# jhhung/kISS

Measured on AMD Instinct MI355X. Metric: bases/sec suffix_sort (chm13v2.0-size synthetic, k=256), higher is better.
Workload: dtype u8; 1 GPU; suffix_sort genome-like synthetic n=3117292070 k=256 (stand-in for chm13v2.0.fa, BASELINE.json configs[1]); PARALLEL_SORTING; text resident in HBM, SA left in HBM; n=3117292070, k=256, seed=2, parallelism=single GPU, lms=905939973, lms_rounds=9, tied_after_round0_item_rounds=184319413, big_segment_item_rounds=72866550, workspace_bytes=80357006484, induce_passes=47

## Files before the change

include/kiss_hip.h:

```cpp
#ifndef KISS_HIP_H
#define KISS_HIP_H

#include <stddef.h>
#include <stdint.h>

#ifdef __cplusplus
extern "C" {
#endif

#define KISS_HIP_VERSION 103

typedef enum kiss_hip_status {
    KISS_HIP_OK = 0,
    KISS_HIP_E_INVALID = -1,
    KISS_HIP_E_NO_DEVICE = -2,
    KISS_HIP_E_HIP = -3,
    KISS_HIP_E_NOMEM = -4,
    KISS_HIP_E_UNSUPPORTED = -5,
    KISS_HIP_E_INTERNAL = -6,
    KISS_HIP_E_IO = -7,
    KISS_HIP_E_DEEP = -8
} kiss_hip_status;

#define KISS_HIP_ALGO_PARALLEL_SORTING 0
// ... 141 lines not shown
                             const uint32_t *splitters, int groups, uint64_t *d_keys_out, uint32_t *d_pos_out,
                             void *stream);
int kiss_hip_stage_sort(kiss_hip_ctx *ctx, const uint64_t *d_keys, const uint32_t *d_pos, uint64_t count, uint64_t n,
                        uint32_t k, uint32_t *d_sorted_out, uint32_t *d_ctx_out, void *stream);
int kiss_hip_stage_induce(kiss_hip_ctx *ctx, uint64_t n, uint32_t k, const uint32_t *d_far_sorted,
                          const uint32_t *d_far_ctx, uint64_t m_far, const uint32_t *d_near_pos, uint64_t near_count,
                          const uint64_t counts12[12], uint32_t *d_SA, void *stream);
int kiss_hip_stage_induce_exact(kiss_hip_ctx *ctx, uint64_t n, uint32_t h0, const uint32_t *d_far_sorted,
                                const uint32_t *d_far_ctx, uint64_t m_far, const uint32_t *d_near_pos, uint64_t near_count,
                                const uint64_t counts12[12], uint32_t *d_SA, void *stream, int *exact_out);
int kiss_hip_stage_refine_exact(kiss_hip_ctx *ctx, uint64_t n, uint32_t h0, uint32_t *d_SA, void *stream);

int kiss_hip_debug_radix_sort(kiss_hip_ctx *ctx, uint64_t *keys, uint32_t *pos, uint64_t count, int key_lo_bit);
int kiss_hip_debug_scan_u32(kiss_hip_ctx *ctx, uint32_t *data, uint64_t count);
int kiss_hip_debug_fail_alloc_over(kiss_hip_ctx *ctx, uint64_t bytes);
int kiss_hip_debug_splitters(const uint64_t *hist, uint64_t bins, int groups, uint32_t *splitters_out,
                             uint64_t *group_counts_out);

typedef struct kiss_hip_fmi_view {
    uint64_t n_sa;
    uint32_t cnt[4];
    uint32_t pri;
    uint32_t sa_intv;
    const uint8_t *bwt;
    const uint32_t *occ1;
    const uint8_t *occ2;
    const uint32_t *sa;
    const uint64_t *b;
    const uint32_t *b_occ;
} kiss_hip_fmi_view;
// ... 180 lines not shown
```

kiss_amd/_lib.py:

```python
import ctypes
import os

_HERE = os.path.dirname(os.path.abspath(__file__))
LIB_PATH = os.path.join(_HERE, "libkiss_hip.so")
HOOKS_LIB_PATH = os.path.join(_HERE, "libkiss_hip_hooks.so")

KISS_HIP_OK = 0
KISS_HIP_E_INVALID, KISS_HIP_E_NO_DEVICE, KISS_HIP_E_HIP, KISS_HIP_E_NOMEM = -1, -2, -3, -4
KISS_HIP_E_UNSUPPORTED, KISS_HIP_E_INTERNAL, KISS_HIP_E_IO, KISS_HIP_E_DEEP = -5, -6, -7, -8
ALGO_PARALLEL_SORTING = 0
ALGO_PREFIX_DOUBLING = 1
MAX_N = 4294963200
VIEW_LOCAL_KEYS, VIEW_LOCAL_POS, VIEW_PART_KEYS, VIEW_PART_POS, VIEW_SORTED, VIEW_SORTED_CTX = range(6)

KERNEL_CLASSES = [
    "pack", "classify", "radix_hist", "radix_scatter", "scan", "keygather", "flag_compact",
    "place", "induce_count", "induce_scatter", "induce_small", "fm_query", "fm_build", "segrank",
    "group_heads", "isa",
]


class Stats(ctypes.Structure):
    _fields_ = [
        ("n", ctypes.c_uint64), ("m", ctypes.c_uint64), ("k", ctypes.c_uint32), ("depth", ctypes.c_uint32),
# ... 202 lines not shown
    lib.kiss_hip_ctx_create_sized.argtypes = [ctypes.POINTER(vp), ctypes.c_int, ctypes.c_uint64, ctypes.c_uint64]
    lib.kiss_hip_ctx_release_io_buffers.argtypes = [vp]
    ip = ctypes.POINTER(ctypes.c_int)
    lib.kiss_hip_multi_create.argtypes = [ctypes.POINTER(vp), ip, ctypes.c_int, ctypes.c_uint64]
    lib.kiss_hip_multi_destroy.argtypes = [vp]
    lib.kiss_hip_multi_suffix_sort_dna_u32.argtypes = [vp, vp, ctypes.c_uint64, ctypes.c_uint32, ctypes.c_int, vp]
    lib.kiss_hip_multi_suffix_sort_dna_u32_dev.argtypes = [vp, vp, ctypes.c_uint64, ctypes.c_uint32, ctypes.c_int, vp]
    lib.kiss_hip_multi_get_stats.argtypes = [vp, ctypes.POINTER(MultiStats)]
    lib.kiss_hip_multi_ctx.argtypes = [vp, ctypes.c_int]
    lib.kiss_hip_multi_ctx.restype = vp
    lib.kiss_hip_suffix_sort_dna_u32_multi.argtypes = [vp, ctypes.c_uint64, ctypes.c_uint32, ctypes.c_int, vp, ip, ctypes.c_int]
    lib.kiss_hip_stage_view.argtypes = [vp, ctypes.c_int, ctypes.POINTER(vp), ctypes.POINTER(ctypes.c_uint64)]
    lib.kiss_hip_stage_reserve.argtypes = [vp, ctypes.c_uint64]
    lib.kiss_hip_debug_fail_alloc_over.argtypes = [vp, ctypes.c_uint64]
    lib.kiss_hip_debug_fail_alloc_over.restype = ctypes.c_int
    lib.kiss_hip_debug_splitters.argtypes = [vp, ctypes.c_uint64, ctypes.c_int, vp, vp]
    lib.kiss_hip_debug_splitters.restype = ctypes.c_int
    lib.kiss_hip_ctx_destroy.argtypes = [vp]
    lib.kiss_hip_ctx_set_profiling.argtypes = [vp, ctypes.c_int]
    lib.kiss_hip_ctx_set_profiling_mask.argtypes = [vp, ctypes.c_uint64]
    lib.kiss_hip_last_hip_error.argtypes = [vp, ctypes.POINTER(ctypes.c_char_p)]
    lib.kiss_hip_get_stats.argtypes = [vp, ctypes.POINTER(Stats)]
    lib.kiss_hip_ctx_workspace_bytes.argtypes = [vp, ctypes.POINTER(ctypes.c_uint64)]
    lib.kiss_hip_suffix_sort_dna_u32.argtypes = [u8p, ctypes.c_uint64, ctypes.c_uint32, ctypes.c_int, vp, ctypes.c_int]
    lib.kiss_hip_ctx_suffix_sort_dna_u32.argtypes = [vp, u8p, ctypes.c_uint64, ctypes.c_uint32, ctypes.c_int, vp]
    lib.kiss_hip_ctx_suffix_sort_dna_u32_dev.argtypes = [vp, vp, ctypes.c_uint64, ctypes.c_uint32, ctypes.c_int, vp, vp]
    lib.kiss_hip_ctx_get_stage_outputs.argtypes = [vp, vp, vp, vp]
    lib.kiss_hip_ctx_verify_sa_dev.argtypes = [vp, vp, ctypes.c_uint64, ctypes.c_uint32, vp, ctypes.POINTER(VerifyReport), vp]
    lib.kiss_hip_ctx_verify_sa_dev.restype = ctypes.c_int
    lib.kiss_hip_sa_digest_host.argtypes = [vp, ctypes.c_uint64]
# ... 100 lines not shown
    "kiss_hip_version", "kiss_hip_strerror", "kiss_hip_device_count", "kiss_hip_ctx_create", "kiss_hip_ctx_destroy",
    "kiss_hip_ctx_set_profiling", "kiss_hip_ctx_set_profiling_mask", "kiss_hip_last_hip_error", "kiss_hip_get_stats", "kiss_hip_ctx_workspace_bytes",
    "kiss_hip_suffix_sort_dna_u32", "kiss_hip_ctx_suffix_sort_dna_u32", "kiss_hip_ctx_suffix_sort_dna_u32_dev",
    "kiss_hip_ctx_get_stage_outputs", "kiss_hip_ctx_verify_sa_dev", "kiss_hip_sa_digest_host", "kiss_hip_fnv1a64_host",
    "kiss_hip_fmi_query_batch_dev", "kiss_hip_fmi_build_dev",
    "kiss_hip_debug_radix_sort", "kiss_hip_debug_scan_u32",
    "kiss_hip_stage_classify", "kiss_hip_stage_local_lms", "kiss_hip_stage_key_hist", "kiss_hip_stage_partition",
    "kiss_hip_stage_sort", "kiss_hip_stage_induce", "kiss_hip_stage_induce_exact", "kiss_hip_stage_refine_exact",
    "kiss_hip_fmi_sizes_for", "kiss_hip_fmi_build_host", "kiss_hip_fmi_query_batch_host",
    "kiss_hip_file_size", "kiss_hip_ctx_parse_text_dev", "kiss_hip_ctx_load_text_file", "kiss_hip_copy_to_host",
    "kiss_hip_free_dev", "kiss_hip_alloc_dev", "kiss_hip_suffix_sort_u8", "kiss_hip_ctx_suffix_sort_u8_dev",
    "kiss_hip_ctx_create_sized", "kiss_hip_ctx_release_io_buffers", "kiss_hip_stage_view", "kiss_hip_stage_reserve",
    "kiss_hip_multi_create", "kiss_hip_multi_destroy", "kiss_hip_multi_suffix_sort_dna_u32",
    "kiss_hip_multi_suffix_sort_dna_u32_dev", "kiss_hip_multi_get_stats", "kiss_hip_multi_ctx",
    "kiss_hip_suffix_sort_dna_u32_multi", "kiss_hip_debug_splitters", "kiss_hip_debug_fail_alloc_over",
    "kiss_hip_has_hooks", "kiss_hip_release_cached_contexts", "kiss_hip_get_stats_sized",
    "kiss_hip_fmi_sizes_ex_for", "kiss_hip_fmi_build_ex_dev", "kiss_hip_fmi_query_ex_dev", "kiss_hip_fmi_build_ex_host",
    "kiss_hip_fmi_query_ex_host", "kiss_hip_ctx_lcp_dna_u32_dev", "kiss_hip_ctx_lcp_u8_dev", "kiss_hip_lcp_dna_u32",
    "kiss_hip_lcp_u8", "kiss_hip_fmi_query_mm_dev", "kiss_hip_fmi_query_mm_host",
    "kiss_hip_fmi8_sizes_for", "kiss_hip_fmi8_build_dev", "kiss_hip_fmi8_build_host", "kiss_hip_fmi8_query_dev",
    "kiss_hip_fmi8_query_host", "kiss_hip_fmi_seeds_dev", "kiss_hip_fmi_seeds_host",
    "kiss_hip_fmi_chain_dev", "kiss_hip_fmi_chain_host",
]
```

kiss_amd/csrc/api.hip:

```cpp
#include "kiss_internal.hpp"
#include <cstdlib>
#include <chrono>
#include <mutex>
#include <cstring>
#include <new>

KTimer::KTimer(kiss_hip_ctx *c, int cls, uint64_t items) : ctx(c), idx(-1)
{
    if (!((ctx->profile_mask >> cls) & 1ull)) return;
    if (ctx->ev_used == ctx->ev_pool.size()) {
        kiss_hip_ctx::Ev e;
        if (hipEventCreate(&e.a) != hipSuccess || hipEventCreate(&e.b) != hipSuccess) return;
        e.cls = 0;
        ctx->ev_pool.push_back(e);
    }
    idx = (int)ctx->ev_used++;
    ctx->ev_pool[idx].cls = cls;
    ctx->stats.launches_kernel[cls]++;
    ctx->stats.items_kernel[cls] += items;
    (void)hipEventRecord(ctx->ev_pool[idx].a, ctx->stream);
}
KTimer::~KTimer()
{
    if (idx >= 0) (void)hipEventRecord(ctx->ev_pool[idx].b, ctx->stream);
// ... 22 lines not shown
    return e ? strtoull(e, nullptr, 0) : dflt;
}
void kiss_opts_refresh(kiss_hip_ctx *ctx)
{
    KissOpts o;
    kiss_opts_supported_from_env(o);
    if (const char *e = getenv("KISS_HIP_SYNC_READBACK")) o.sync_readback = atoi(e) != 0;
    o.no_serialize = env_on("KISS_HIP_NO_SERIALIZE");
    o.no_lms_exact = env_on("KISS_HIP_NO_LMS_EXACT");
    o.heads_by_compare = env_on("KISS_HIP_LMS_HEADS_BY_COMPARE");
    o.no_early_out = env_on("KISS_HIP_NO_EARLY_OUT");
    o.no_pivot_rounds = env_on("KISS_HIP_NO_PIVOT_ROUNDS");
    o.pivot_from_round2 = env_on("KISS_HIP_PIVOT_FROM_ROUND2");
    o.pair_keys = env_on("KISS_HIP_PAIR_KEYS");
    o.no_fc0_onepass = env_on("KISS_HIP_NO_FC0_ONEPASS");
    o.no_pair_records = env_on("KISS_HIP_NO_PAIR_RECORDS");
    o.no_class_bytes = env_on("KISS_HIP_NO_CLASS_BYTES");
    o.no_pivot_ctx = env_on("KISS_HIP_NO_PIVOT_CTX");
    o.no_taint = env_on("KISS_HIP_NO_TAINT");
    o.isa_direct = env_on("KISS_HIP_ISA_DIRECT");
    o.no_onesweep = env_on("KISS_HIP_NO_ONESWEEP");
    o.rx_one_tile = env_on("KISS_HIP_RX_ONE_TILE");
    o.merge_lms = env_on("KISS_HIP_MERGE_LMS");
    o.no_small_alphabet = env_on("KISS_HIP_NO_SMALL_ALPHABET");
    o.induce_one_pass = env_on("KISS_HIP_INDUCE_ONE_PASS");
    o.verify = env_on("KISS_HIP_VERIFY");
    o.no_prefault = env_on("KISS_HIP_NO_PREFAULT");
    o.doubling_h0 = (uint32_t)env_u64("KISS_HIP_DOUBLING_H0", 0);
    o.tcap0 = env_u64("KISS_HIP_TCAP0", 0);
    o.pivot_slots = (int)env_u64("KISS_HIP_PIVOT_SLOTS", 3);
// ... 212 lines not shown
        if (ctx->opts.doubling_h0 >= 32 && ctx->opts.doubling_h0 <= (1u << 20)) h0 = ctx->opts.doubling_h0;
        if (n < 4ull * h0 + 1024) h0 = 0;
        else {
            k = h0;
            depth = (uint64_t)KISS_STRIDE * ((uint64_t)k / KISS_STRIDE + 1);
        }
    }
    ctx->stats.refine_depth = h0;

    hipEvent_t ev[8];
    for (auto &e : ev) KCHECK(hipEventCreate(&e));
    const bool lms_exact = !ctx->opts.no_lms_exact;
    int rc = KISS_HIP_OK;
    for (int attempt = 0; attempt < 2; attempt++) {
        (void)hipEventRecord(ev[0], ctx->stream);
        if ((rc = kiss_pack_text(ctx, d_S, n))) break;
        (void)hipEventRecord(ev[1], ctx->stream);
        if ((rc = kiss_classify(ctx, n, depth, 0, n))) break;
        (void)hipEventRecord(ev[2], ctx->stream);
        ctx->hfar = nullptr;
        ctx->h_depth = h0;
        if (h0 && lms_exact && ctx->m_far && !ctx->opts.heads_by_compare) {
            if ((rc = kiss_need_ctx_words(ctx))) break;
            const uint64_t hwords = (ctx->m_far + 8 + 3) / 4;
            ctx->hfar = reinterpret_cast<uint8_t *>(ctx->CTX + ((n + 2 - hwords) & ~3ull));
            if ((rc = kiss_fill_u32(ctx, ctx->hfar, 0x01010101u, (ctx->m_far + 3) / 4))) break;
        }
        rc = kiss_lms_sort(ctx, n, k, depth);
        if (rc == KISS_INTERNAL_TOO_DEEP && attempt == 0 && n >= 4ull * KISS_EXACT_H0 + 1024) {
            (void)hipStreamSynchronize(ctx->stream);
            h0 = KISS_EXACT_H0;
// ... 533 lines not shown
    return KISS_HIP_OK;
}

int kiss_hip_debug_fail_alloc_over(kiss_hip_ctx *ctx, uint64_t bytes)
{
    if (!ctx) return KISS_HIP_E_INVALID;
#ifdef KISS_HIP_HOOKS
    ctx->fail_alloc_over = bytes;
    return KISS_HIP_OK;
#else
    (void)bytes;
    return KISS_HIP_E_UNSUPPORTED;
#endif
}

int kiss_hip_has_hooks(void)
{
#ifdef KISS_HIP_HOOKS
    return 1;
#else
    return 0;
#endif
}

int kiss_hip_debug_scan_u32(kiss_hip_ctx *ctx, uint32_t *data, uint64_t count)
{
    if (!ctx || !data || count > ctx->m_cap) return KISS_HIP_E_INVALID;
    KCHECK(hipSetDevice(ctx->device));
    ctx->stream = ctx->own_stream;
    KCHECK(hipMemcpy(ctx->posA, data, count * 4, hipMemcpyHostToDevice));
// ... 42 lines not shown
```

kiss_amd/csrc/classify.hip:

```cpp
#include "kiss_internal.hpp"

namespace {

constexpr uint64_t HI = 0xAAAAAAAAAAAAAAAAull;
constexpr uint64_t LO = 0x5555555555555555ull;
constexpr int CL_THREADS = 256;

__global__ __launch_bounds__(256) void k_pack(const uint8_t *__restrict__ S, uint64_t n, uint64_t *__restrict__ pk,
                                              uint64_t words)
{
    uint64_t w = (uint64_t)blockIdx.x * blockDim.x + threadIdx.x;
    if (w >= words) return;
    uint64_t base = w * 32;
    uint64_t out = 0;
    if (base + 32 <= n && ((reinterpret_cast<uintptr_t>(S + base) & 15u) == 0)) {
        const uint4 *p = reinterpret_cast<const uint4 *>(S + base);
        uint4 v0 = p[0], v1 = p[1];
        uint32_t q[8] = {v0.x, v0.y, v0.z, v0.w, v1.x, v1.y, v1.z, v1.w};
#pragma unroll
        for (int t = 0; t < 8; t++) {
            uint32_t u = q[t] & 0x03030303u;
            uint32_t r = ((u & 0x3u) << 6) | (((u >> 8) & 0x3u) << 4) | (((u >> 16) & 0x3u) << 2) | ((u >> 24) & 0x3u);
            out |= (uint64_t)r << (56 - 8 * t);
        }
    } else {
        for (int j = 0; j < 32; j++) {
            uint64_t i = base + j;
            uint64_t c = (i < n) ? (uint64_t)(S[i] & 3u) : 0ull;
            out |= c << (62 - 2 * j);
        }
    }
    pk[w] = out;
}

struct WordMasks {
    uint64_t x;
    uint64_t A;
    uint64_t B;
};

__device__ __forceinline__ WordMasks word_masks(const uint64_t *__restrict__ pk, uint64_t w, uint64_t n, uint64_t words)
{
    WordMasks m;
    const uint64_t x = w < words ? pk[w] : 0ull;
    uint64_t nx = __shfl_down(x, 1, 64);
    if (lane_id() == 63) nx = w + 1 < words ? pk[w + 1] : 0ull;
    if (w >= words) {
        m.x = 0;
        m.A = LO;
        m.B = 0;
        return m;
    }
    uint64_t y = (x << 2) | (nx >> 62);
    uint64_t d = x ^ y;
    uint64_t eqh = ~d & HI;
    uint64_t eql = ~d & LO;
    uint64_t eq = eqh & (eql << 1);
    uint64_t xy = ~x & y;
    uint64_t lt = (xy & HI) | (eqh & ((xy & LO) << 1));
    int64_t rem = (int64_t)(n - 1) - (int64_t)(w * 32);
    uint64_t vmask = rem >= 32 ? ~0ull : (rem <= 0 ? 0ull : (~0ull << (64 - 2 * rem)));
    lt &= vmask;
    eq &= vmask;
    m.x = x;
    m.A = lt | eq | LO;
    m.B = lt;
    return m;
}

__device__ __forceinline__ uint32_t word_carry(uint64_t A, uint64_t B, uint32_t cin, uint64_t *sum)
{
    uint64_t s = A + B;
    uint32_t c1 = s < A;
    uint64_t s2 = s + cin;
    uint32_t c2 = s2 < s;
    *sum = s2;
    return c1 | c2;
}

__device__ __forceinline__ uint32_t wave_carry(uint32_t G, uint32_t P, uint32_t wave_cin, uint32_t *wave_cout)
{
    uint64_t gm = __ballot(G != 0);
    uint64_t pm = __ballot(P != 0);
    uint64_t rg = __brevll(gm), rp = __brevll(pm);
// ... 56 lines not shown
    if (lane_id() == 0) {
        lds[wave * 2 + 0] = wc0;
        lds[wave * 2 + 1] = wc1 & ~wc0;
    }
    __syncthreads();
    if (threadIdx.x == 0) {
        uint32_t a = 0, b = 1;
        for (int v = CL_THREADS / 64 - 1; v >= 0; v--) {
            a = lds[v * 2] | (lds[v * 2 + 1] & a);
            b = lds[v * 2] | (lds[v * 2 + 1] & b);
        }
        tile_gp[blockIdx.x] = a | ((b & ~a) << 1);
    }
}

__global__ __launch_bounds__(1024) void k_tile_cin(uint32_t *__restrict__ tile_gp, uint64_t tiles)
{
    __shared__ uint32_t sg[1024], sp[1024], scin[1024];
    const uint64_t chunk = (tiles + 1023) / 1024;
    const uint64_t beg = (uint64_t)threadIdx.x * chunk;
    const uint64_t end = beg + chunk < tiles ? beg + chunk : tiles;
    uint32_t a = 0, b = 1;
    for (uint64_t t = end; t > beg; t--) {
        uint32_t gp = tile_gp[t - 1];
        uint32_t g = gp & 1u, p = (gp >> 1) & 1u;
        a = g | (p & a);
        b = g | (p & b);
    }
    if (beg >= end) { a = 0; b = 1; }
    sg[threadIdx.x] = a;
    sp[threadIdx.x] = b & ~a;
    __syncthreads();
    if (threadIdx.x == 0) {
        uint32_t c = 0;
        for (int i = 1023; i >= 0; i--) {
            scin[i] = c;
            c = sg[i] | (sp[i] & c);
        }
    }
    __syncthreads();
    uint32_t c = scin[threadIdx.x];
    for (uint64_t t = end; t > beg; t--) {
        uint32_t gp = tile_gp[t - 1];
        tile_gp[t - 1] = c;
        c = (gp & 1u) | (((gp >> 1) & 1u) & c);
    }
}

constexpr int TC_CHUNK = 16;
__global__ __launch_bounds__(256) void k_tile_cin_chunks(const uint32_t *__restrict__ tile_gp, uint64_t tiles, uint64_t chunks,
                                                         uint32_t *__restrict__ chunk_gp)
{
    const uint64_t c = (uint64_t)blockIdx.x * 256 + threadIdx.x;
    if (c >= chunks) return;
    const uint64_t beg = c * TC_CHUNK, end = beg + TC_CHUNK < tiles ? beg + TC_CHUNK : tiles;
    uint32_t a = 0, b = 1;
    for (uint64_t t = end; t > beg; t--) {
        const uint32_t gp = tile_gp[t - 1];
        const uint32_t g = gp & 1u, p = (gp >> 1) & 1u;
        a = g | (p & a);
        b = g | (p & b);
    }
    chunk_gp[c] = a | ((b & ~a) << 1);
}

__global__ __launch_bounds__(256) void k_tile_cin_apply(uint32_t *__restrict__ tile_gp, uint64_t tiles, uint64_t chunks,
                                                        const uint32_t *__restrict__ chunk_cin)
{
    const uint64_t ch = (uint64_t)blockIdx.x * 256 + threadIdx.x;
    if (ch >= chunks) return;
    const uint64_t beg = ch * TC_CHUNK, end = beg + TC_CHUNK < tiles ? beg + TC_CHUNK : tiles;
    uint32_t gp[TC_CHUNK];
#pragma unroll
    for (int e = 0; e < TC_CHUNK; e++) gp[e] = beg + e < end ? tile_gp[beg + e] : 0u;
    uint32_t c = chunk_cin[ch];
#pragma unroll
    for (int e = TC_CHUNK - 1; e >= 0; e--) {
        if (beg + e < end) {
            tile_gp[beg + e] = c;
            c = (gp[e] & 1u) | (((gp[e] >> 1) & 1u) & c);
        }
    }
}

template <bool EMIT>
__global__ __launch_bounds__(CL_THREADS) void k_classify(const uint64_t *__restrict__ pk, uint64_t n, uint64_t words,
                                                        uint64_t tiles, const uint32_t *__restrict__ tile_cin,
                                                        uint32_t *__restrict__ tile_cnt,
                                                        uint32_t *__restrict__ d_counts, uint64_t far_limit,
                                                        uint64_t win_lo, uint64_t win_hi,
                                                        uint64_t tile_lo, uint64_t tile_hi,
                                                        uint32_t *__restrict__ lms_pos, uint64_t *__restrict__ lms_key,
                                                        uint32_t *__restrict__ ghist,
                                                        uint32_t *__restrict__ part)
{
    __shared__ uint32_t hh[EMIT ? KISS_R0_PASSES * 256 : 1];
    if (EMIT && ghist) {
// ... 131 lines not shown
            uint32_t v = acc[i];
#pragma unroll
            for (int d = 32; d >= 1; d >>= 1) v += __shfl_xor(v, d, 64);
            if (lane_id() == 0) wacc[threadIdx.x >> 6][i] = v;
        }
        __syncthreads();
        if (threadIdx.x < 16) {
            uint32_t v = 0;
            if (threadIdx.x < 13)
                for (int wv = 0; wv < CL_THREADS / 64; wv++) v += wacc[wv][threadIdx.x];
            part[(uint64_t)blockIdx.x * 16 + threadIdx.x] = v;
        }
    }
}

__global__ __launch_bounds__(256) void k_sum_rows(const uint32_t *__restrict__ part, uint32_t rows, uint32_t cols,
                                                  uint32_t *__restrict__ out)
{
    const uint32_t c = blockIdx.x * 256 + threadIdx.x;
    if (c >= cols) return;
    const uint32_t per = (rows + gridDim.y - 1) / gridDim.y;
    const uint32_t r0 = blockIdx.y * per, r1 = r0 + per < rows ? r0 + per : rows;
    uint32_t v = 0;
#pragma unroll 8
    for (uint32_t r = r0; r < r1; r++) v += part[(uint64_t)r * cols + c];
    if (v) atomicAdd(&out[c], v);
}

}

int kiss_pack_text(kiss_hip_ctx *ctx, const uint8_t *d_S, uint64_t n)
{
    const uint64_t words = div_up(n, 32) + 4;
    if (words > ctx->pk_words) return KINTERNAL();
    KTimer t(ctx, KISS_HIP_K_PACK, n);
    hipLaunchKernelGGL(k_pack, dim3((unsigned)div_up(words, 256)), dim3(256), 0, ctx->stream, d_S, n, ctx->pk, words);
    KCHECK(hipGetLastError());
    return KISS_HIP_OK;
}

int kiss_classify(kiss_hip_ctx *ctx, uint64_t n, uint64_t depth, uint64_t win_lo, uint64_t win_hi)
{
    if (win_hi > n) win_hi = n;
    if (win_lo > win_hi) win_lo = win_hi;
    ctx->lms_pos_complete = win_lo == 0 && win_hi == n;
    const uint64_t words = div_up(n, 32);
    const uint64_t tiles = div_up(words, CL_THREADS);
    if (tiles > ctx->n_tiles_cap) return KINTERNAL();
    uint64_t far_limit = ~0ull;
    bool none_far = false;
    if (depth != 0) {
        if (depth > n) none_far = true;
        else far_limit = n - depth;
    }
    constexpr uint64_t TILE_BASES = (uint64_t)CL_THREADS * 32;
    const uint64_t tile_lo = win_lo / TILE_BASES < tiles ? win_lo / TILE_BASES : tiles;
    uint64_t tile_hi = div_up(win_hi, TILE_BASES) < tiles ? div_up(win_hi, TILE_BASES) : tiles;
    if (tile_hi < tile_lo || win_hi <= win_lo) tile_hi = tile_lo;
    const uint64_t wtiles = tile_hi - tile_lo;
    KTRY(kiss_zero_u32(ctx, ctx->d_counts, 16));
    uint32_t *part = ctx->cl_part;
    {
        KTimer t(ctx, KISS_HIP_K_CLASSIFY, n);
        hipLaunchKernelGGL(k_tile_gp, dim3((unsigned)tiles), dim3(CL_THREADS), 0, ctx->stream, ctx->pk, n, words,
                           ctx->tile_gp);
        if (tiles > 4096) {
            const uint64_t chunks = div_up(tiles, TC_CHUNK);
            hipLaunchKernelGGL(k_tile_cin_chunks, dim3((unsigned)div_up(chunks, 256)), dim3(256), 0, ctx->stream, ctx->tile_gp,
                               tiles, chunks, ctx->tile_cnt);
            hipLaunchKernelGGL(k_tile_cin, dim3(1), dim3(1024), 0, ctx->stream, ctx->tile_cnt, chunks);
            hipLaunchKernelGGL(k_tile_cin_apply, dim3((unsigned)div_up(chunks, 256)), dim3(256), 0, ctx->stream, ctx->tile_gp,
                               tiles, chunks, ctx->tile_cnt);
        } else {
            hipLaunchKernelGGL(k_tile_cin, dim3(1), dim3(1024), 0, ctx->stream, ctx->tile_gp, tiles);
        }
        if (wtiles) {
            unsigned grid = (unsigned)(wtiles < 2048 ? wtiles : 2048);
            hipLaunchKernelGGL(k_classify<false>, dim3(grid), dim3(CL_THREADS), 0, ctx->stream, ctx->pk, n, words, tiles,
                               ctx->tile_gp, ctx->tile_cnt, ctx->d_counts, far_limit, win_lo, win_hi, tile_lo, tile_hi,
                               (uint32_t *)nullptr, (uint64_t *)nullptr, (uint32_t *)nullptr, part);
            hipLaunchKernelGGL(k_sum_rows, dim3(1, 32), dim3(256), 0, ctx->stream, part, grid, 16u, ctx->d_counts);
        }
        KCHECK(hipGetLastError());
    }
    if (wtiles) KTRY(kiss_scan_u32(ctx, ctx->tile_cnt + tile_lo, ctx->tile_cnt + tile_lo, wtiles));
    KTRY(kiss_readback(ctx, ctx->d_counts, 16));
    for (int i = 0; i < 12; i++) ctx->counts[i] = ctx->h_pinned[i];
    uint64_t m = (uint64_t)ctx->h_pinned[8] + ctx->h_pinned[9] + ctx->h_pinned[10] + ctx->h_pinned[11];
    ctx->m = m;
// ... 20 lines not shown
```

kiss_amd/csrc/kiss_internal.hpp:

```cpp
#pragma once
#include <hip/hip_runtime.h>
#include <stdint.h>
#include <stddef.h>
#include <mutex>
#include <vector>
#include "../../include/kiss_hip.h"

struct KissOpts {
    bool debug = false;
    int xfer_threads = 0;
    int prefault_threads = 0;
    bool sync_readback = false;
    bool no_lms_exact = false;
    bool heads_by_compare = false;
    bool no_early_out = false;
    bool no_pivot_rounds = false;
    bool pivot_from_round2 = false;
    bool pair_keys = false;
    bool no_fc0_onepass = false;
    bool no_pair_records = false;
    bool no_class_bytes = false;
    bool no_pivot_ctx = false;
    bool no_taint = false;
    bool isa_direct = false;
    bool no_onesweep = false;
    bool rx_one_tile = false;
    bool merge_lms = false;
    bool no_small_alphabet = false;
    bool induce_one_pass = false;
    bool verify = false;
    bool no_prefault = false;
    bool no_serialize = false;
    bool lock_launches = false;
    bool sync_launches = false;
// ... 77 lines not shown
    uint64_t fail_alloc_over = 0;
    uint64_t m_cap0 = 0;
    uint64_t t_cap = 0;
    uint64_t flags_cap = 0;
    uint64_t tied_bytes = 0;
    uint64_t ws_bytes = 0;
    uint64_t lms_bytes = 0;

    uint64_t *pk = nullptr;
    uint64_t pk_words = 0;
    uint32_t *tile_gp = nullptr;
    uint32_t *tile_cnt = nullptr;
    uint8_t *CLS = nullptr;
    uint32_t *cl_part = nullptr;
    uint64_t n_tiles_cap = 0;
    uint32_t *d_counts = nullptr;
    uint32_t *lms_pos = nullptr;
    bool lms_pos_complete = false;
    uint64_t *keyA = nullptr, *keyB = nullptr;
    uint32_t *posA = nullptr, *posB = nullptr;
    uint32_t *segA = nullptr, *segB = nullptr;
    uint32_t *slotA = nullptr, *slotB = nullptr;
    uint32_t *segstartA = nullptr, *segstartB = nullptr;
    uint64_t *bkeyA = nullptr, *bkeyB = nullptr;
    uint32_t *bposA = nullptr, *bposB = nullptr, *bsegA = nullptr, *bsegB = nullptr, *bslot = nullptr;
    uint64_t *flags = nullptr;
    uint32_t *lms_sorted_far = nullptr;
    uint32_t *lms_ctx_far = nullptr;
    uint32_t *lmsP = nullptr;
    uint32_t *lmsC = nullptr;
// ... 64 lines not shown
struct KTimer {
    kiss_hip_ctx *ctx;
    int idx;
    KTimer(kiss_hip_ctx *c, int cls, uint64_t items);
    ~KTimer();
};
void ktimer_collect(kiss_hip_ctx *ctx);

static inline uint64_t div_up(uint64_t a, uint64_t b) { return (a + b - 1) / b; }

int kiss_lms_reserve(kiss_hip_ctx *ctx, uint64_t m_cap, uint64_t t_cap_wanted = 0);
int kiss_tied_reserve(kiss_hip_ctx *ctx, uint64_t t_cap);
int kiss_workspace_ready(kiss_hip_ctx *ctx);
int kiss_need_ctx_words(kiss_hip_ctx *ctx);
int kiss_pack_text(kiss_hip_ctx *ctx, const uint8_t *d_S, uint64_t n);
int kiss_classify(kiss_hip_ctx *ctx, uint64_t n, uint64_t depth , uint64_t win_lo, uint64_t win_hi);
int kiss_readback(kiss_hip_ctx *ctx, const void *d_src, uint32_t nwords);
std::mutex &kiss_device_mutex(int device);
int kiss_scan_u32(kiss_hip_ctx *ctx, const uint32_t *in, uint32_t *out, uint64_t count);
int kiss_scan_u64(kiss_hip_ctx *ctx, const uint64_t *in, uint64_t *out, uint64_t count);
int kiss_zero_u32(kiss_hip_ctx *ctx, void *p, uint64_t count_u32);
int kiss_fill_u32(kiss_hip_ctx *ctx, void *p, uint32_t value, uint64_t count_u32);
struct RadixBufs {
    uint64_t *key[2];
    uint32_t *seg[2];
    uint32_t *pos[2];
    const uint32_t *first_pos = nullptr;
};
int kiss_radix_sort(kiss_hip_ctx *ctx, RadixBufs &b, uint64_t count, int key_lo_bit, int seg_bits, int *result_idx);
int kiss_radix_check(kiss_hip_ctx *ctx);
// ... 89 lines not shown
```

kiss_amd/csrc/scan.hip:

```cpp
#include "kiss_internal.hpp"

namespace {

constexpr int SCAN_THREADS = 256;
constexpr int SCAN_ROWS = 4;
constexpr int SCAN_VEC = 4;
constexpr int SCAN_ROW_ELEMS = SCAN_THREADS * SCAN_VEC;
constexpr int SCAN_BLOCK = SCAN_ROWS * SCAN_ROW_ELEMS;

template <typename T>
__device__ __forceinline__ T wave_inclusive_scan(T v)
{
#pragma unroll
    for (int d = 1; d < 64; d <<= 1) {
        T o = __shfl_up(v, d, 64);
        if ((int)lane_id() >= d) v += o;
    }
    return v;
}

template <typename T>
__device__ __forceinline__ void load_row(const T *__restrict__ in, uint64_t base, uint64_t count, T v[SCAN_VEC])
{
    if (base + SCAN_VEC <= count && ((reinterpret_cast<uintptr_t>(in + base) & (sizeof(T) * SCAN_VEC - 1)) == 0)) {
// ... 71 lines not shown
        for (int w = 0; w < 1024 / 64; w++) {
            T t = lds[w];
            lds[w] = acc;
            acc += t;
        }
    }
    __syncthreads();
    T run = inc - s + lds[wave];
    for (uint64_t i = beg; i < end; i++) {
        T t = data[i];
        data[i] = run;
        run += t;
    }
}

template <typename T, bool ONE_BLOCK>
__global__ __launch_bounds__(SCAN_THREADS) void k_scan_final(const T *in, T *out, uint64_t count,
                                                            const T *__restrict__ blocksums)
{
    __shared__ T wsum[SCAN_ROWS][SCAN_THREADS / 64];
    const int wave = threadIdx.x >> 6;
    const uint64_t bbase = (uint64_t)blockIdx.x * SCAN_BLOCK + (uint64_t)threadIdx.x * SCAN_VEC;
    T v[SCAN_ROWS][SCAN_VEC];
    T c[SCAN_ROWS], inc[SCAN_ROWS];
#pragma unroll
    for (int r = 0; r < SCAN_ROWS; r++) {
        load_row<T>(in, bbase + (uint64_t)r * SCAN_ROW_ELEMS, count, v[r]);
        c[r] = v[r][0] + v[r][1] + v[r][2] + v[r][3];
    }
#pragma unroll
    for (int r = 0; r < SCAN_ROWS; r++) {
        inc[r] = wave_inclusive_scan<T>(c[r]);
        if (lane_id() == 63) wsum[r][wave] = inc[r];
    }
    __syncthreads();
    T run = ONE_BLOCK ? (T)0 : blocksums[blockIdx.x];
#pragma unroll
    for (int r = 0; r < SCAN_ROWS; r++) {
        T pre = run;
#pragma unroll
        for (int w = 0; w < SCAN_THREADS / 64; w++) {
            T t = wsum[r][w];
            if (w < wave) pre += t;
            run += t;
        }
        pre += inc[r] - c[r];
        T o[SCAN_VEC];
        o[0] = pre;
        o[1] = o[0] + v[r][0];
        o[2] = o[1] + v[r][1];
        o[3] = o[2] + v[r][2];
        store_row<T>(out, bbase + (uint64_t)r * SCAN_ROW_ELEMS, count, o);
    }
}

template <typename T>
int scan_impl(kiss_hip_ctx *ctx, const T *in, T *out, uint64_t count)
{
    if (count == 0) return KISS_HIP_OK;
    const uint64_t nb = div_up(count, SCAN_BLOCK);
    if (nb > ctx->scan_tmp_cap) return KINTERNAL();
    T *bs = reinterpret_cast<T *>(ctx->scan_tmp);
    KTimer t(ctx, KISS_HIP_K_SCAN, count);
    if (nb == 1) {
        hipLaunchKernelGGL((k_scan_final<T, true>), dim3(1), dim3(SCAN_THREADS), 0, ctx->stream, in, out, count, (const T *)nullptr);
        KCHECK(hipGetLastError());
        return KISS_HIP_OK;
    }
    hipLaunchKernelGGL(k_scan_reduce<T>, dim3((unsigned)nb), dim3(SCAN_THREADS), 0, ctx->stream, in, count, bs);
    hipLaunchKernelGGL(k_scan_single<T>, dim3(1), dim3(1024), 0, ctx->stream, bs, nb);
    hipLaunchKernelGGL((k_scan_final<T, false>), dim3((unsigned)nb), dim3(SCAN_THREADS), 0, ctx->stream, in, out, count, bs);
    KCHECK(hipGetLastError());
    return KISS_HIP_OK;
}

}

__global__ void k_zero_u32(uint32_t *p, uint64_t count)
{
    uint64_t i = (uint64_t)blockIdx.x * blockDim.x + threadIdx.x;
    if (i < count) p[i] = 0;
}
int kiss_zero_u32(kiss_hip_ctx *ctx, void *p, uint64_t count_u32)
{
    if (!count_u32) return KISS_HIP_OK;
    hipLaunchKernelGGL(k_zero_u32, dim3((unsigned)div_up(count_u32, 256)), dim3(256), 0, ctx->stream, (uint32_t *)p,
// ... 36 lines not shown
```

Baseline: 43.40 billion bases/s.

## Fuse text packing with tile carry and class counting; two-launch small scans

Adds a k_pack_count kernel that packs the text and, in the same pass, computes per-tile carry/propagate words, LMS counts and class histograms. The later classify step can then skip the separate k_tile_gp pass and the per-tile count pass, and only does carry resolution with delta corrections. The aim is to cut a full read of the packed text and several launches from the front end. Separately, scans with at most 1024 blocks now sum the raw block totals inside the final kernel and skip the single-block scan launch. This adds intricate boundary and carry bookkeeping that must match the unfused path exactly.

```diff
diff --git a/include/kiss_hip.h b/include/kiss_hip.h
--- a/include/kiss_hip.h
+++ b/include/kiss_hip.h
@@ -179,6 +179,7 @@
 int kiss_hip_debug_radix_sort(kiss_hip_ctx *ctx, uint64_t *keys, uint32_t *pos, uint64_t count, int key_lo_bit);
 int kiss_hip_debug_scan_u32(kiss_hip_ctx *ctx, uint32_t *data, uint64_t count);
 int kiss_hip_debug_fail_alloc_over(kiss_hip_ctx *ctx, uint64_t bytes);
+int kiss_hip_debug_front_form(kiss_hip_ctx *ctx);
 int kiss_hip_debug_splitters(const uint64_t *hist, uint64_t bins, int groups, uint32_t *splitters_out,
                              uint64_t *group_counts_out);
 
diff --git a/kiss_amd/_lib.py b/kiss_amd/_lib.py
--- a/kiss_amd/_lib.py
+++ b/kiss_amd/_lib.py
@@ -240,6 +240,9 @@
     lib.kiss_hip_stage_reserve.argtypes = [vp, ctypes.c_uint64]
     lib.kiss_hip_debug_fail_alloc_over.argtypes = [vp, ctypes.c_uint64]
     lib.kiss_hip_debug_fail_alloc_over.restype = ctypes.c_int
+    if hasattr(lib, "kiss_hip_debug_front_form"):
+        lib.kiss_hip_debug_front_form.argtypes = [vp]
+        lib.kiss_hip_debug_front_form.restype = ctypes.c_int
     lib.kiss_hip_debug_splitters.argtypes = [vp, ctypes.c_uint64, ctypes.c_int, vp, vp]
     lib.kiss_hip_debug_splitters.restype = ctypes.c_int
     lib.kiss_hip_ctx_destroy.argtypes = [vp]
@@ -370,6 +373,7 @@
     "kiss_hip_multi_create", "kiss_hip_multi_destroy", "kiss_hip_multi_suffix_sort_dna_u32",
     "kiss_hip_multi_suffix_sort_dna_u32_dev", "kiss_hip_multi_get_stats", "kiss_hip_multi_ctx",
     "kiss_hip_suffix_sort_dna_u32_multi", "kiss_hip_debug_splitters", "kiss_hip_debug_fail_alloc_over",
+    "kiss_hip_debug_front_form",
     "kiss_hip_has_hooks", "kiss_hip_release_cached_contexts", "kiss_hip_get_stats_sized",
     "kiss_hip_fmi_sizes_ex_for", "kiss_hip_fmi_build_ex_dev", "kiss_hip_fmi_query_ex_dev", "kiss_hip_fmi_build_ex_host",
     "kiss_hip_fmi_query_ex_host", "kiss_hip_ctx_lcp_dna_u32_dev", "kiss_hip_ctx_lcp_u8_dev", "kiss_hip_lcp_dna_u32",
diff --git a/kiss_amd/csrc/api.hip b/kiss_amd/csrc/api.hip
--- a/kiss_amd/csrc/api.hip
+++ b/kiss_amd/csrc/api.hip
@@ -60,6 +60,7 @@
     o.pivot_from_round2 = env_on("KISS_HIP_PIVOT_FROM_ROUND2");
     o.pair_keys = env_on("KISS_HIP_PAIR_KEYS");
     o.no_fc0_onepass = env_on("KISS_HIP_NO_FC0_ONEPASS");
+    o.no_fused_front = env_on("KISS_HIP_NO_FUSED_FRONT");
     o.no_pair_records = env_on("KISS_HIP_NO_PAIR_RECORDS");
     o.no_class_bytes = env_on("KISS_HIP_NO_CLASS_BYTES");
     o.no_pivot_ctx = env_on("KISS_HIP_NO_PIVOT_CTX");
@@ -302,7 +303,7 @@
     int rc = KISS_HIP_OK;
     for (int attempt = 0; attempt < 2; attempt++) {
         (void)hipEventRecord(ev[0], ctx->stream);
-        if ((rc = kiss_pack_text(ctx, d_S, n))) break;
+        if ((rc = kiss_pack_text_counted(ctx, d_S, n, depth))) break;
         (void)hipEventRecord(ev[1], ctx->stream);
         if ((rc = kiss_classify(ctx, n, depth, 0, n))) break;
         (void)hipEventRecord(ev[2], ctx->stream);
@@ -866,6 +867,16 @@
 #endif
 }
 
+int kiss_hip_debug_front_form(kiss_hip_ctx *ctx)
+{
+    if (!ctx) return KISS_HIP_E_INVALID;
+#ifdef KISS_HIP_HOOKS
+    return ctx->front_form;
+#else
+    return KISS_HIP_E_UNSUPPORTED;
+#endif
+}
+
 int kiss_hip_has_hooks(void)
 {
 #ifdef KISS_HIP_HOOKS
diff --git a/kiss_amd/csrc/classify.hip b/kiss_amd/csrc/classify.hip
--- a/kiss_amd/csrc/classify.hip
+++ b/kiss_amd/csrc/classify.hip
@@ -6,11 +6,9 @@
 constexpr uint64_t LO = 0x5555555555555555ull;
 constexpr int CL_THREADS = 256;
 
-__global__ __launch_bounds__(256) void k_pack(const uint8_t *__restrict__ S, uint64_t n, uint64_t *__restrict__ pk,
-                                              uint64_t words)
-{
-    uint64_t w = (uint64_t)blockIdx.x * blockDim.x + threadIdx.x;
-    if (w >= words) return;
+template <bool ROLLED = false>
+__device__ __forceinline__ uint64_t pack_word(const uint8_t *__restrict__ S, uint64_t n, uint64_t w)
+{
     uint64_t base = w * 32;
     uint64_t out = 0;
     if (base + 32 <= n && ((reinterpret_cast<uintptr_t>(S + base) & 15u) == 0)) {
@@ -23,6 +21,13 @@
             uint32_t r = ((u & 0x3u) << 6) | (((u >> 8) & 0x3u) << 4) | (((u >> 16) & 0x3u) << 2) | ((u >> 24) & 0x3u);
             out |= (uint64_t)r << (56 - 8 * t);
         }
+    } else if (ROLLED) {
+#pragma unroll 1
+        for (int j = 0; j < 32; j++) {
+            uint64_t i = base + j;
+            uint64_t c = (i < n) ? (uint64_t)(S[i] & 3u) : 0ull;
+            out |= c << (62 - 2 * j);
+        }
     } else {
         for (int j = 0; j < 32; j++) {
             uint64_t i = base + j;
@@ -30,7 +35,15 @@
             out |= c << (62 - 2 * j);
         }
     }
-    pk[w] = out;
+    return out;
+}
+
+__global__ __launch_bounds__(256) void k_pack(const uint8_t *__restrict__ S, uint64_t n, uint64_t *__restrict__ pk,
+                                              uint64_t words)
+{
+    uint64_t w = (uint64_t)blockIdx.x * blockDim.x + threadIdx.x;
+    if (w >= words) return;
+    pk[w] = pack_word(S, n, w);
 }
 
 struct WordMasks {
@@ -39,12 +52,9 @@
     uint64_t B;
 };
 
-__device__ __forceinline__ WordMasks word_masks(const uint64_t *__restrict__ pk, uint64_t w, uint64_t n, uint64_t words)
+__device__ __forceinline__ WordMasks masks_of(uint64_t x, uint64_t nx, uint64_t w, uint64_t n, uint64_t words)
 {
     WordMasks m;
-    const uint64_t x = w < words ? pk[w] : 0ull;
-    uint64_t nx = __shfl_down(x, 1, 64);
-    if (lane_id() == 63) nx = w + 1 < words ? pk[w + 1] : 0ull;
     if (w >= words) {
         m.x = 0;
         m.A = LO;
@@ -68,6 +78,14 @@
     return m;
 }
 
+__device__ __forceinline__ WordMasks word_masks(const uint64_t *__restrict__ pk, uint64_t w, uint64_t n, uint64_t words)
+{
+    const uint64_t x = w < words ? pk[w] : 0ull;
+    uint64_t nx = __shfl_down(x, 1, 64);
+    if (lane_id() == 63) nx = w + 1 < words ? pk[w + 1] : 0ull;
+    return masks_of(x, nx, w, n, words);
+}
+
 __device__ __forceinline__ uint32_t word_carry(uint64_t A, uint64_t B, uint32_t cin, uint64_t *sum)
 {
     uint64_t s = A + B;
@@ -154,7 +172,39 @@
     }
 }
 
-__global__ __launch_bounds__(1024) void k_tile_cin(uint32_t *__restrict__ tile_gp, uint64_t tiles)
+constexpr uint32_t TD_R_SHIFT = 2;
+constexpr uint32_t TD_R_MASK = 0x3FFFu;
+constexpr uint32_t TD_C_SHIFT = 16;
+constexpr uint32_t TD_LMS = 1u << 18;
+constexpr uint32_t TD_FAR = 1u << 19;
+
+__device__ __forceinline__ void delta_apply(uint32_t gp, uint32_t cin, uint32_t *__restrict__ tile_cnt_entry, uint32_t acc[9])
+{
+    const uint32_t r = (gp >> TD_R_SHIFT) & TD_R_MASK;
+    if (!cin || !r) return;
+    const uint32_t c = (gp >> TD_C_SHIFT) & 3u;
+    const uint32_t l = (gp & TD_LMS) ? 1u : 0u;
+#pragma unroll
+    for (uint32_t k = 0; k < 4; k++) {
+        acc[k] += c == k ? r : 0u;
+        acc[4 + k] += c == k ? l : 0u;
+    }
+    acc[8] += (gp & TD_FAR) ? 1u : 0u;
+    if (l) *tile_cnt_entry += 1u;
+}
+__device__ __forceinline__ void delta_flush(const uint32_t acc[9], uint32_t *__restrict__ d_counts)
+{
+#pragma unroll
+    for (int i = 0; i < 9; i++) {
+        uint32_t v = acc[i];
+#pragma unroll
+        for (int d = 32; d >= 1; d >>= 1) v += __shfl_xor(v, d, 64);
+        if (lane_id() == 0 && v) atomicAdd(&d_counts[4 + i], v);
+    }
+}
+
+__global__ __launch_bounds__(1024) void k_tile_cin(uint32_t *__restrict__ tile_gp, uint64_t tiles,
+                                                   uint32_t *__restrict__ tile_cnt, uint32_t *__restrict__ d_counts)
 {
     __shared__ uint32_t sg[1024], sp[1024], scin[1024];
     const uint64_t chunk = (tiles + 1023) / 1024;
@@ -180,11 +230,14 @@
     }
     __syncthreads();
     uint32_t c = scin[threadIdx.x];
+    uint32_t acc[9] = {0, 0, 0, 0, 0, 0, 0, 0, 0};
     for (uint64_t t = end; t > beg; t--) {
         uint32_t gp = tile_gp[t - 1];
         tile_gp[t - 1] = c;
+        if (d_counts) delta_apply(gp, c, &tile_cnt[t - 1], acc);
         c = (gp & 1u) | (((gp >> 1) & 1u) & c);
     }
+    if (d_counts) delta_flush(acc, d_counts);
 }
 
 constexpr int TC_CHUNK = 16;
@@ -205,22 +258,27 @@
 }
 
 __global__ __launch_bounds__(256) void k_tile_cin_apply(uint32_t *__restrict__ tile_gp, uint64_t tiles, uint64_t chunks,
-                                                        const uint32_t *__restrict__ chunk_cin)
+                                                        const uint32_t *__restrict__ chunk_cin,
+                                                        uint32_t *__restrict__ tile_cnt, uint32_t *__restrict__ d_counts)
 {
     const uint64_t ch = (uint64_t)blockIdx.x * 256 + threadIdx.x;
-    if (ch >= chunks) return;
-    const uint64_t beg = ch * TC_CHUNK, end = beg + TC_CHUNK < tiles ? beg + TC_CHUNK : tiles;
-    uint32_t gp[TC_CHUNK];
-#pragma unroll
-    for (int e = 0; e < TC_CHUNK; e++) gp[e] = beg + e < end ? tile_gp[beg + e] : 0u;
-    uint32_t c = chunk_cin[ch];
-#pragma unroll
-    for (int e = TC_CHUNK - 1; e >= 0; e--) {
-        if (beg + e < end) {
-            tile_gp[beg + e] = c;
-            c = (gp[e] & 1u) | (((gp[e] >> 1) & 1u) & c);
-        }
-    }
+    uint32_t acc[9] = {0, 0, 0, 0, 0, 0, 0, 0, 0};
+    if (ch < chunks) {
+        const uint64_t beg = ch * TC_CHUNK, end = beg + TC_CHUNK < tiles ? beg + TC_CHUNK : tiles;
+        uint32_t gp[TC_CHUNK];
+#pragma unroll
+        for (int e = 0; e < TC_CHUNK; e++) gp[e] = beg + e < end ? tile_gp[beg + e] : 0u;
+        uint32_t c = chunk_cin[ch];
+#pragma unroll
+        for (int e = TC_CHUNK - 1; e >= 0; e--) {
+            if (beg + e < end) {
+                tile_gp[beg + e] = c;
+                if (d_counts) delta_apply(gp[e], c, &tile_cnt[beg + e], acc);
+                c = (gp[e] & 1u) | (((gp[e] >> 1) & 1u) & c);
+            }
+        }
+    }
+    if (d_counts) delta_flush(acc, d_counts);
 }
 
 template <bool EMIT>
@@ -382,6 +440,136 @@
     }
 }
 
+__global__ __launch_bounds__(CL_THREADS) void k_pack_count(const uint8_t *__restrict__ S, uint64_t n, uint64_t *__restrict__ pk,
+                                                          uint64_t pwords, uint64_t words, uint64_t tiles, uint64_t far_limit,
+                                                          uint32_t *__restrict__ tile_gp, uint32_t *__restrict__ tile_cnt,
+                                                          uint32_t *__restrict__ part)
+{
+    constexpr int WAVES = CL_THREADS / 64;
+    __shared__ uint32_t wgp[WAVES];
+    __shared__ uint32_t wrun[WAVES];
+    __shared__ uint32_t wsum[WAVES];
+    __shared__ uint32_t edge[2];
+    const uint32_t lane = lane_id(), wave = threadIdx.x >> 6;
+    uint32_t acc[13];
+#pragma unroll
+    for (int i = 0; i < 13; i++) acc[i] = 0;
+
+    for (uint64_t tile = blockIdx.x; tile < tiles; tile += gridDim.x) {
+        const uint64_t w = tile * CL_THREADS + threadIdx.x;
+        const uint64_t x = pack_word<true>(S, n, w);
+        if (w < pwords) pk[w] = x;
+        if (tile == tiles - 1 && threadIdx.x < 4) {
+            const uint64_t v = tiles * CL_THREADS + threadIdx.x;
+            if (v < pwords) pk[v] = 0;
+        }
+        uint64_t nx = __shfl_down(x, 1, 64);
+        if (lane == 63) nx = (w + 1) * 32 < n ? (uint64_t)(S[(w + 1) * 32] & 3u) << 62 : 0ull;
+        uint32_t pb = __shfl_up((uint32_t)x, 1, 64) & 3u;
+        if (lane == 0) pb = (w > 0 && w * 32 - 1 < n) ? S[w * 32 - 1] & 3u : 0u;
+
+        const WordMasks m = masks_of(x, nx, w, n, words);
+        uint64_t sum;
+        const uint32_t c0 = word_carry(m.A, m.B, 0, &sum);
+        const uint32_t c1 = word_carry(m.A, m.B, 1, &sum);
+        const uint32_t G = c0, P = c1 & ~c0;
+        uint32_t wc0, wc1;
+        (void)wave_carry(G, P, 0, &wc0);
+        (void)wave_carry(G, P, 1, &wc1);
+        const uint64_t npm = ~__ballot(P != 0);
+        const uint32_t nfull = npm ? (uint32_t)__clzll((long long)npm) : 64u;
+        const uint64_t neq = ~((m.A & HI & ~m.B) | LO);
+        const uint32_t te = neq ? (uint32_t)__builtin_ctzll(neq) >> 1 : 0u;
+        const uint32_t info = te | ((uint32_t)(x >> (2u * te)) & 3u) << 8;
+        const uint32_t sinfo = __shfl(info, (int)((63u - nfull) & 63u), 64);
+        if (lane == 0) {
+            wgp[wave] = wc0 | ((wc1 & ~wc0) << 1);
+            wrun[wave] = nfull == 64u ? (64u * 32u) | (1u << 16) : (nfull * 32u + (sinfo & 0xFFu)) | ((sinfo >> 8) << 17);
+        }
+        if (threadIdx.x == 0) edge[0] = pb;
+        if (threadIdx.x == CL_THREADS - 1) edge[1] = (uint32_t)x & 3u;
+        __syncthreads();
+        uint32_t c = 0;
+        for (int v = WAVES - 1; v > (int)wave; v--) c = (wgp[v] & 1u) | ((wgp[v] >> 1) & c);
+        uint32_t dummy;
+        const uint32_t cin = wave_carry(G, P, c, &dummy);
+        const uint32_t cout = word_carry(m.A, m.B, cin, &sum);
+        uint64_t T = ((~sum & LO) >> 2) | ((uint64_t)cout << 62);
+        const int64_t b = (int64_t)n - (int64_t)(w * 32);
+        const uint64_t V = b >= 32 ? LO : (b <= 0 ? 0ull : (LO & (~0ull << (64 - 2 * b))));
+        T &= V;
+        const uint64_t lmsmask = T & (gt_prev_mask(m.x, (uint64_t)pb) >> 1);
+        const uint64_t hi = (m.x >> 1) & LO, lo = m.x & LO;
+        const uint64_t is[4] = {~hi & ~lo & LO, ~hi & lo, hi & ~lo, hi & lo};
+#pragma unroll
+        for (int k = 0; k < 4; k++) {
+            acc[k] += __popcll(is[k] & V);
+            acc[4 + k] += __popcll(is[k] & T);
+            acc[8 + k] += __popcll(is[k] & lmsmask);
+        }
+        uint64_t farmask = lmsmask;
+        if (far_limit != ~0ull) {
+            const int64_t fj = (int64_t)far_limit - (int64_t)(w * 32);
+            farmask = fj >= 31 ? lmsmask : (fj < 0 ? 0ull : (lmsmask & (~0ull << (62 - 2 * fj))));
+        }
+        acc[12] += __popcll(farmask);
+        uint32_t v = __popcll(lmsmask);
+#pragma unroll
+        for (int d = 32; d >= 1; d >>= 1) v += __shfl_xor(v, d, 64);
+        if (lane == 0) wsum[wave] = v;
+        if (threadIdx.x == 0) {
+            uint32_t ca = 0, cb = 1;
+            for (int u = WAVES - 1; u >= 0; u--) {
+                ca = (wgp[u] & 1u) | ((wgp[u] >> 1) & ca);
+                cb = (wgp[u] & 1u) | ((wgp[u] >> 1) & cb);
+            }
+            uint32_t r = 0, prev = edge[0];
+            bool has_prev = tile > 0;
+            for (int u = WAVES - 1; u >= 0; u--) {
+                const uint32_t wr = wrun[u];
+                r += wr & 0xFFFFu;
+                if (!((wr >> 16) & 1u)) {
+                    prev = (wr >> 17) & 3u;
+                    has_prev = true;
+                    break;
+                }
+            }
+            const uint32_t ch = edge[1];
+            uint32_t word = ca | ((cb & ~ca) << 1);
+            if (r) {
+                word |= (r << TD_R_SHIFT) | (ch << TD_C_SHIFT);
+                if (has_prev && prev > ch) {
+                    word |= TD_LMS;
+                    const uint64_t f = (tile + 1) * (uint64_t)(CL_THREADS * 32) - r;
+                    if (f <= far_limit) word |= TD_FAR;
+                }
+            }
+            tile_gp[tile] = word;
+        }
+        __syncthreads();
+        if (threadIdx.x == 0) {
+            uint32_t t = 0;
+            for (int i = 0; i < WAVES; i++) t += wsum[i];
+            tile_cnt[tile] = t;
+        }
+    }
+    __shared__ uint32_t wacc[WAVES][16];
+#pragma unroll
+    for (int i = 0; i < 13; i++) {
+        uint32_t v = acc[i];
+#pragma unroll
+        for (int d = 32; d >= 1; d >>= 1) v += __shfl_xor(v, d, 64);
+        if (lane == 0) wacc[wave][i] = v;
+    }
+    __syncthreads();
+    if (threadIdx.x < 16) {
+        uint32_t v = 0;
+        if (threadIdx.x < 13)
+            for (int wv = 0; wv < WAVES; wv++) v += wacc[wv][threadIdx.x];
+        part[(uint64_t)blockIdx.x * 16 + threadIdx.x] = v;
+    }
+}
+
 __global__ __launch_bounds__(256) void k_sum_rows(const uint32_t *__restrict__ part, uint32_t rows, uint32_t cols,
                                                   uint32_t *__restrict__ out)
 {
@@ -401,9 +589,42 @@
 {
     const uint64_t words = div_up(n, 32) + 4;
     if (words > ctx->pk_words) return KINTERNAL();
+    ctx->front_valid = false;
     KTimer t(ctx, KISS_HIP_K_PACK, n);
     hipLaunchKernelGGL(k_pack, dim3((unsigned)div_up(words, 256)), dim3(256), 0, ctx->stream, d_S, n, ctx->pk, words);
     KCHECK(hipGetLastError());
+    return KISS_HIP_OK;
+}
+
+static void far_limit_of(uint64_t n, uint64_t depth, uint64_t *far_limit, bool *none_far)
+{
+    *far_limit = ~0ull;
+    *none_far = false;
+    if (depth != 0) {
+        if (depth > n) *none_far = true;
+        else *far_limit = n - depth;
+    }
+}
+
+int kiss_pack_text_counted(kiss_hip_ctx *ctx, const uint8_t *d_S, uint64_t n, uint64_t depth)
+{
+    const uint64_t cwords = div_up(n, 32), tiles = div_up(cwords, CL_THREADS);
+    if (ctx->opts.no_fused_front || n == 0 || tiles > ctx->n_tiles_cap) return kiss_pack_text(ctx, d_S, n);
+    const uint64_t words = cwords + 4;
+    if (words > ctx->pk_words) return KINTERNAL();
+    uint64_t far_limit;
+    bool none_far;
+    far_limit_of(n, depth, &far_limit, &none_far);
+    ctx->front_valid = false;
+    const unsigned grid = (unsigned)(tiles < 8192 ? tiles : 8192);
+    KTimer t(ctx, KISS_HIP_K_PACK, n);
+    hipLaunchKernelGGL(k_pack_count, dim3(grid), dim3(CL_THREADS), 0, ctx->stream, d_S, n, ctx->pk, words, cwords, tiles,
+                       far_limit, ctx->tile_gp, ctx->tile_cnt, ctx->cl_part);
+    KCHECK(hipGetLastError());
+    ctx->front_valid = true;
+    ctx->front_n = n;
+    ctx->front_depth = depth;
+    ctx->front_rows = grid;
     return KISS_HIP_OK;
 }
 
@@ -415,20 +636,37 @@
     const uint64_t words = div_up(n, 32);
     const uint64_t tiles = div_up(words, CL_THREADS);
     if (tiles > ctx->n_tiles_cap) return KINTERNAL();
-    uint64_t far_limit = ~0ull;
-    bool none_far = false;
-    if (depth != 0) {
-        if (depth > n) none_far = true;
-        else far_limit = n - depth;
-    }
+    uint64_t far_limit;
+    bool none_far;
+    far_limit_of(n, depth, &far_limit, &none_far);
     constexpr uint64_t TILE_BASES = (uint64_t)CL_THREADS * 32;
     const uint64_t tile_lo = win_lo / TILE_BASES < tiles ? win_lo / TILE_BASES : tiles;
     uint64_t tile_hi = div_up(win_hi, TILE_BASES) < tiles ? div_up(win_hi, TILE_BASES) : tiles;
     if (tile_hi < tile_lo || win_hi <= win_lo) tile_hi = tile_lo;
     const uint64_t wtiles = tile_hi - tile_lo;
+    const bool fused = ctx->front_valid && ctx->front_n == n && ctx->front_depth == depth && win_lo == 0 && win_hi == n;
+    ctx->front_valid = false;
+    ctx->front_form = fused ? 1 : 0;
     KTRY(kiss_zero_u32(ctx, ctx->d_counts, 16));
     uint32_t *part = ctx->cl_part;
-    {
+    if (fused) {
+        KTimer t(ctx, KISS_HIP_K_CLASSIFY, n);
+        hipLaunchKernelGGL(k_sum_rows, dim3(1, 32), dim3(256), 0, ctx->stream, part, ctx->front_rows, 16u, ctx->d_counts);
+        if (tiles > 4096) {
+            const uint64_t chunks = div_up(tiles, TC_CHUNK);
+            uint32_t *chunk_gp = part + 8192ull * 16;
+            hipLaunchKernelGGL(k_tile_cin_chunks, dim3((unsigned)div_up(chunks, 256)), dim3(256), 0, ctx->stream, ctx->tile_gp,
+                               tiles, chunks, chunk_gp);
+            hipLaunchKernelGGL(k_tile_cin, dim3(1), dim3(1024), 0, ctx->stream, chunk_gp, chunks, (uint32_t *)nullptr,
+                               (uint32_t *)nullptr);
+            hipLaunchKernelGGL(k_tile_cin_apply, dim3((unsigned)div_up(chunks, 256)), dim3(256), 0, ctx->stream, ctx->tile_gp,
+                               tiles, chunks, chunk_gp, ctx->tile_cnt, ctx->d_counts);
+        } else {
+            hipLaunchKernelGGL(k_tile_cin, dim3(1), dim3(1024), 0, ctx->stream, ctx->tile_gp, tiles, ctx->tile_cnt,
+                               ctx->d_counts);
+        }
+        KCHECK(hipGetLastError());
+    } else {
         KTimer t(ctx, KISS_HIP_K_CLASSIFY, n);
         hipLaunchKernelGGL(k_tile_gp, dim3((unsigned)tiles), dim3(CL_THREADS), 0, ctx->stream, ctx->pk, n, words,
                            ctx->tile_gp);
@@ -436,11 +674,13 @@
             const uint64_t chunks = div_up(tiles, TC_CHUNK);
             hipLaunchKernelGGL(k_tile_cin_chunks, dim3((unsigned)div_up(chunks, 256)), dim3(256), 0, ctx->stream, ctx->tile_gp,
                                tiles, chunks, ctx->tile_cnt);
-            hipLaunchKernelGGL(k_tile_cin, dim3(1), dim3(1024), 0, ctx->stream, ctx->tile_cnt, chunks);
+            hipLaunchKernelGGL(k_tile_cin, dim3(1), dim3(1024), 0, ctx->stream, ctx->tile_cnt, chunks, (uint32_t *)nullptr,
+                               (uint32_t *)nullptr);
             hipLaunchKernelGGL(k_tile_cin_apply, dim3((unsigned)div_up(chunks, 256)), dim3(256), 0, ctx->stream, ctx->tile_gp,
-                               tiles, chunks, ctx->tile_cnt);
+                               tiles, chunks, ctx->tile_cnt, (uint32_t *)nullptr, (uint32_t *)nullptr);
         } else {
-            hipLaunchKernelGGL(k_tile_cin, dim3(1), dim3(1024), 0, ctx->stream, ctx->tile_gp, tiles);
+            hipLaunchKernelGGL(k_tile_cin, dim3(1), dim3(1024), 0, ctx->stream, ctx->tile_gp, tiles, (uint32_t *)nullptr,
+                               (uint32_t *)nullptr);
         }
         if (wtiles) {
             unsigned grid = (unsigned)(wtiles < 2048 ? wtiles : 2048);
diff --git a/kiss_amd/csrc/kiss_internal.hpp b/kiss_amd/csrc/kiss_internal.hpp
--- a/kiss_amd/csrc/kiss_internal.hpp
+++ b/kiss_amd/csrc/kiss_internal.hpp
@@ -18,6 +18,7 @@
     bool pivot_from_round2 = false;
     bool pair_keys = false;
     bool no_fc0_onepass = false;
+    bool no_fused_front = false;
     bool no_pair_records = false;
     bool no_class_bytes = false;
     bool no_pivot_ctx = false;
@@ -125,6 +126,10 @@
     uint8_t *CLS = nullptr;
     uint32_t *cl_part = nullptr;
     uint64_t n_tiles_cap = 0;
+    bool front_valid = false;
+    uint64_t front_n = 0, front_depth = 0;
+    uint32_t front_rows = 0;
+    int front_form = 0;
     uint32_t *d_counts = nullptr;
     uint32_t *lms_pos = nullptr;
     bool lms_pos_complete = false;
@@ -219,6 +224,7 @@
 int kiss_workspace_ready(kiss_hip_ctx *ctx);
 int kiss_need_ctx_words(kiss_hip_ctx *ctx);
 int kiss_pack_text(kiss_hip_ctx *ctx, const uint8_t *d_S, uint64_t n);
+int kiss_pack_text_counted(kiss_hip_ctx *ctx, const uint8_t *d_S, uint64_t n, uint64_t depth);
 int kiss_classify(kiss_hip_ctx *ctx, uint64_t n, uint64_t depth , uint64_t win_lo, uint64_t win_hi);
 int kiss_readback(kiss_hip_ctx *ctx, const void *d_src, uint32_t nwords);
 std::mutex &kiss_device_mutex(int device);
diff --git a/kiss_amd/csrc/scan.hip b/kiss_amd/csrc/scan.hip
--- a/kiss_amd/csrc/scan.hip
+++ b/kiss_amd/csrc/scan.hip
@@ -7,6 +7,8 @@
 constexpr int SCAN_VEC = 4;
 constexpr int SCAN_ROW_ELEMS = SCAN_THREADS * SCAN_VEC;
 constexpr int SCAN_BLOCK = SCAN_ROWS * SCAN_ROW_ELEMS;
+constexpr unsigned SCAN_TWO_LAUNCH_BLOCKS = 1024;
+enum ScanForm { SCAN_ONE_BLOCK, SCAN_SUMS_SCANNED, SCAN_SUMS_RAW };
 
 template <typename T>
 __device__ __forceinline__ T wave_inclusive_scan(T v)
@@ -109,12 +111,16 @@
     }
 }
 
-template <typename T, bool ONE_BLOCK>
+template <typename T, int FORM>
 __global__ __launch_bounds__(SCAN_THREADS) void k_scan_final(const T *in, T *out, uint64_t count,
                                                             const T *__restrict__ blocksums)
 {
     __shared__ T wsum[SCAN_ROWS][SCAN_THREADS / 64];
+    __shared__ T bsum[SCAN_THREADS / 64];
     const int wave = threadIdx.x >> 6;
+    T before = 0;
+    if (FORM == SCAN_SUMS_RAW)
+        for (uint32_t b = threadIdx.x; b < blockIdx.x; b += SCAN_THREADS) before += blocksums[b];
     const uint64_t bbase = (uint64_t)blockIdx.x * SCAN_BLOCK + (uint64_t)threadIdx.x * SCAN_VEC;
     T v[SCAN_ROWS][SCAN_VEC];
     T c[SCAN_ROWS], inc[SCAN_ROWS];
@@ -128,8 +134,16 @@
         inc[r] = wave_inclusive_scan<T>(c[r]);
         if (lane_id() == 63) wsum[r][wave] = inc[r];
     }
-    __syncthreads();
-    T run = ONE_BLOCK ? (T)0 : blocksums[blockIdx.x];
+    if (FORM == SCAN_SUMS_RAW) {
+#pragma unroll
+        for (int d = 32; d >= 1; d >>= 1) before += __shfl_xor(before, d, 64);
+        if (lane_id() == 0) bsum[wave] = before;
+    }
+    __syncthreads();
+    T run = 0;
+    if (FORM == SCAN_SUMS_SCANNED) run = blocksums[blockIdx.x];
+    if (FORM == SCAN_SUMS_RAW)
+        for (int w = 0; w < SCAN_THREADS / 64; w++) run += bsum[w];
 #pragma unroll
     for (int r = 0; r < SCAN_ROWS; r++) {
         T pre = run;
@@ -158,13 +172,17 @@
     T *bs = reinterpret_cast<T *>(ctx->scan_tmp);
     KTimer t(ctx, KISS_HIP_K_SCAN, count);
     if (nb == 1) {
-        hipLaunchKernelGGL((k_scan_final<T, true>), dim3(1), dim3(SCAN_THREADS), 0, ctx->stream, in, out, count, (const T *)nullptr);
+        hipLaunchKernelGGL((k_scan_final<T, SCAN_ONE_BLOCK>), dim3(1), dim3(SCAN_THREADS), 0, ctx->stream, in, out, count, (const T *)nullptr);
         KCHECK(hipGetLastError());
         return KISS_HIP_OK;
     }
     hipLaunchKernelGGL(k_scan_reduce<T>, dim3((unsigned)nb), dim3(SCAN_THREADS), 0, ctx->stream, in, count, bs);
-    hipLaunchKernelGGL(k_scan_single<T>, dim3(1), dim3(1024), 0, ctx->stream, bs, nb);
-    hipLaunchKernelGGL((k_scan_final<T, false>), dim3((unsigned)nb), dim3(SCAN_THREADS), 0, ctx->stream, in, out, count, bs);
+    if (nb <= SCAN_TWO_LAUNCH_BLOCKS) {
+        hipLaunchKernelGGL((k_scan_final<T, SCAN_SUMS_RAW>), dim3((unsigned)nb), dim3(SCAN_THREADS), 0, ctx->stream, in, out, count, bs);
+    } else {
+        hipLaunchKernelGGL(k_scan_single<T>, dim3(1), dim3(1024), 0, ctx->stream, bs, nb);
+        hipLaunchKernelGGL((k_scan_final<T, SCAN_SUMS_SCANNED>), dim3((unsigned)nb), dim3(SCAN_THREADS), 0, ctx->stream, in, out, count, bs);
+    }
     KCHECK(hipGetLastError());
     return KISS_HIP_OK;
 }
```

Result: no change. 43.78 billion bases/s, median of 6 (+0.9%).
